# enijkamp/apex_example

Hardware: AMD Instinct MI355X
Metric: images/sec (whole node) ResNet-50 amp O2 (higher is better)
Workload: dtype bf16; 1 GPU; model=resnet50, global_batch=256, per_gpu_batch=256, image_size=224, parallelism=dp1, impl=amd, opt_level=O2, optimizer=FusedSGD(momentum=0.9, wd=5e-5), channels_last=True, fused_bn=True, syncbn=False, force_collectives=False, gemm_1x1=True, hip_graph=False, main_stream_priority=default, deterministic=False

## Files before the change

apex_example_amd/ops/pool.py:

```python
from __future__ import annotations


import torch
import torch.nn as nn
import torch.nn.functional as F

from .. import _native

_FUSE_STEM = True
_FUSE_STEM_BWD = True
_GAP_KERNEL = True


class MaxPool2dNHWCFunction(torch.autograd.Function):
    @staticmethod
    def forward(ctx, x, k, s, p):
        y, idx = _native.require().pool.max_fwd(x, k, s, p)
        ctx.save_for_backward(idx)
        ctx.geom = (x.size(2), x.size(3), k, s, p)
        return y

    @staticmethod
    def backward(ctx, dy):
        (idx,) = ctx.saved_tensors
        H, W, k, s, p = ctx.geom
        return _native.require().pool.max_bwd(dy, idx, H, W, k, s, p), None, None, None


class BNReLUMaxPoolFunction(torch.autograd.Function):

    @staticmethod
    def forward(ctx, x, weight, bias, running_mean, running_var, nbt, eps, momentum, k, s, p,
                pg=None, slab=None, shift=None):
        C = _native.require()
        inv_total = None
        count = x.numel() // x.size(1)
        if pg is None and slab is not None:
            mean, invstd = C.bn.slab_train_stats(slab, count, shift, running_mean, running_var,
                                                 nbt, float(eps), float(momentum))
        elif pg is None:
            mean, invstd = C.bn.train_stats(x, running_mean, running_var, nbt, float(eps),
                                            float(momentum))
        else:
            import torch.distributed as dist
            world = dist.get_world_size(pg)
            packed = (C.bn.slab_packed_stats(slab, count, shift) if slab is not None
                      else C.bn.local_stats_packed(x))
            gathered = torch.empty(world * packed.numel(), dtype=packed.dtype, device=x.device)
            if dist.get_backend(pg) == "nccl":
                dist.all_gather_into_tensor(gathered, packed, group=pg)
            else:
                dist.all_gather(list(gathered.chunk(world)), packed, group=pg)
            mean, invstd, inv_total = C.bn.combine_stats_sync(
                gathered.view(world, -1), float(eps), float(momentum), running_mean,
                running_var, nbt)
        y, idx = C.pool.max_fwd_bn(x, mean, invstd, weight, bias, k, s, p)
        ctx.save_for_backward(x, weight, bias, mean, invstd, idx)
        ctx.geom = (x.size(2), x.size(3), k, s, p)
        ctx.pg, ctx.inv_total = pg, inv_total
        return y

    @staticmethod
    def backward(ctx, dy):
        x, weight, bias, mean, invstd, idx = ctx.saved_tensors
        H, W, k, s, p = ctx.geom
        C = _native.require()
        need_w = weight is not None and (ctx.needs_input_grad[1] or ctx.needs_input_grad[2])
        if (ctx.pg is None and _FUSE_STEM_BWD and (k, s, p) == (3, 2, 1) and x.size(1) == 64
                and x.element_size() == 2 and dy.dtype == x.dtype):
            dbn, slab = C.pool.max_bwd_bn(dy, idx, H, W, x, mean, invstd, weight, bias)
            sum_dy, sum_dy_xmu, gw, gb = C.bn.slab_reduce_grad(slab, invstd, weight, need_w)
            count = float(x.numel() // x.size(1))
        elif ctx.pg is None:
            dbn = C.pool.max_bwd(dy, idx, H, W, k, s, p)
            sum_dy, sum_dy_xmu, gw, gb = C.bn.reduce_grad(dbn, x, mean, invstd, weight, bias,
                                                          None, True, need_w)
            count = float(x.numel() // x.size(1))
        else:
            import torch.distributed as dist
            dbn = C.pool.max_bwd(dy, idx, H, W, k, s, p)
            sum_dy, sum_dy_xmu, gw, gb = C.bn.reduce_grad(dbn, x, mean, invstd, weight, bias,
                                                          None, True, need_w,
                                                          sum_scale=ctx.inv_total)
            n = sum_dy.numel()
            dist.all_reduce(sum_dy.as_strided((2 * n,), (1,)), group=ctx.pg)
            count = 1.0
        dx, _ = C.bn.backward_elemt(dbn, x, mean, invstd, weight, bias, sum_dy, sum_dy_xmu,
                                    count, None, True, False)
        return (dx, gw if need_w else None, gb if need_w else None,
                None, None, None, None, None, None, None, None, None, None, None)


def _stem_pg(bn):
    from .batch_norm import BatchNorm2dReLU

    if type(bn) is BatchNorm2dReLU:
        return None
    from ..parallel.sync_batchnorm import SyncBatchNorm, syncbn_comm_group
    import torch.distributed as dist

    if type(bn) is not SyncBatchNorm or bn.channel_last:
        return False
# ... 71 lines not shown
```

csrc/hip/pool.hip:

```cpp
#include <cstdlib>

#include "amd_dev.h"
#include "amd_kernels.h"
#include "bn_common.h"

namespace amd {

namespace {

constexpr int kPoolThreads = 256;
constexpr int kPoolBNMaxC = 512;

struct PoolBN {
  const float *mean, *invstd, *w, *b;
};

template <typename T, bool VEC, bool BN>
__global__ void __launch_bounds__(kPoolThreads)
    maxpool_fwd_k(const T* __restrict__ x, T* __restrict__ y, uint8_t* __restrict__ idx,
                  int N, int H, int W, int C, int OH, int OW, int k, int s, int p, PoolBN bn) {
  constexpr int V = VEC ? 8 : 1;
  const int CV = C / V;
  const int64_t total = (int64_t)N * OH * OW * CV;
  for (int64_t t = (int64_t)blockIdx.x * blockDim.x + threadIdx.x; t < total;
// ... 182 lines not shown
    for (int i = 0; i < 8; ++i) {
      best[i] = -INFINITY;
      arg[i] = first;
    }
#pragma unroll
    for (int tap = 0; tap < 9; ++tap) {
      if (!((okm >> tap) & 1u)) continue;
      float v[8];
      unpack8_any<T>(raw[tap], v);
      if constexpr (BN) {
#pragma unroll
        for (int i = 0; i < 8; ++i) v[i] = to_f32(from_f32<T>(fmaxf(fmaf(v[i], sc[i], sh[i]), 0.f)));
      }
#pragma unroll
      for (int i = 0; i < 8; ++i) {
        if (v[i] > best[i] || (v[i] != v[i] && best[i] == best[i])) {
          best[i] = v[i];
          arg[i] = tap;
        }
      }
    }
    const int64_t o = (((int64_t)n * OH + oh) * OW + ow) * C + cv * 8;
    store8(y + o, best);
    uint32_t lo = 0, hi = 0;
#pragma unroll
    for (int i = 0; i < 4; ++i) {
      lo |= (uint32_t)(arg[i] & 0xff) << (8 * i);
      hi |= (uint32_t)(arg[i + 4] & 0xff) << (8 * i);
    }
    *reinterpret_cast<uint2*>(idx + o) = make_uint2(lo, hi);
  }
}

template <typename T, bool BNR = false>
__global__ void __launch_bounds__(kPoolThreads)
    maxpool3s2_bwd2_k(const T* __restrict__ dy, const uint8_t* __restrict__ idx,
                      T* __restrict__ dx, int N, int H, int W, int C, int OH, int OW,
                      const T* __restrict__ xin = nullptr, const float* __restrict__ mean = nullptr,
                      const float* __restrict__ invstd = nullptr,
                      const float* __restrict__ bw = nullptr, const float* __restrict__ bb = nullptr,
                      float* __restrict__ slab = nullptr) {
  static_assert(sizeof(T) == 2, "16-bit activations");
  const int CV = C / 8, BH = (H + 1) / 2, BW = (W + 1) / 2;
  const int64_t total = (int64_t)N * BH * BW * CV;
  float mu[8], sc[8], sh[8], s1[8], s2[8];
  if constexpr (BNR) {
    const int cg = (int)(((int64_t)blockIdx.x * blockDim.x + threadIdx.x) % CV);
#pragma unroll
    for (int c = 0; c < 8; ++c) {
      const int ch = cg * 8 + c;
      mu[c] = mean[ch];
      chan_affine(mean, invstd, bw ? bw[ch] : 1.f, bb ? bb[ch] : 0.f, ch, sc[c], sh[c]);
      s1[c] = s2[c] = 0.f;
    }
  }
  for (int64_t t = (int64_t)blockIdx.x * blockDim.x + threadIdx.x; t < total;
       t += (int64_t)gridDim.x * blockDim.x) {
    const int cv = (int)(t % CV);
    int64_t pix = t / CV;
    const int j = (int)(pix % BW);
    pix /= BW;
    const int i = (int)(pix % BH);
    const int n = (int)(pix / BH);
    float g[4][8];
    uint32_t wd[4][2];
    bool ok[4];
#pragma unroll
    for (int a = 0; a < 2; ++a)
#pragma unroll
      for (int b = 0; b < 2; ++b) {
        const int q = a * 2 + b;
        ok[q] = i + a < OH && j + b < OW;
        const int64_t o = (((int64_t)n * OH + (ok[q] ? i + a : i)) * OW + (ok[q] ? j + b : j)) * C +
                          cv * 8;
        unpack8_any<T>(*reinterpret_cast<const p_u32x4*>(dy + o), g[q]);
        const uint2 w2 = *reinterpret_cast<const uint2*>(idx + o);
        wd[q][0] = w2.x;
        wd[q][1] = w2.y;
      }
    auto tap_of = [&](int q, int c) { return (int)((wd[q][c >> 2] >> (8 * (c & 3))) & 0xff); };
#pragma unroll
    for (int dh = 0; dh < 2; ++dh) {
      const int h = 2 * i + dh;
      if (h >= H) continue;
#pragma unroll
      for (int dw = 0; dw < 2; ++dw) {
        const int w = 2 * j + dw;
        if (w >= W) continue;
        float acc[8];
#pragma unroll
        for (int c = 0; c < 8; ++c) acc[c] = 0.f;
#pragma unroll
        for (int a = 0; a < 2; ++a) {
          if (a == 1 && dh == 0) continue;
          const int kh = dh == 0 ? 1 : (a == 0 ? 2 : 0);
#pragma unroll
          for (int b = 0; b < 2; ++b) {
            if (b == 1 && dw == 0) continue;
            const int kw = dw == 0 ? 1 : (b == 0 ? 2 : 0);
            const int q = a * 2 + b;
            if (!ok[q]) continue;
#pragma unroll
            for (int c = 0; c < 8; ++c)
              if (tap_of(q, c) == kh * 3 + kw) acc[c] += g[q][c];
          }
        }
        const int64_t o = (((int64_t)n * H + h) * W + w) * C + cv * 8;
        store8(dx + o, acc);
        if constexpr (BNR) {
          float xv[8];
          unpack8_any<T>(*reinterpret_cast<const p_u32x4*>(xin + o), xv);
#pragma unroll
          for (int c = 0; c < 8; ++c) {
            const float g = to_f32(from_f32<T>(acc[c]));
            const float d = fmaf(xv[c], sc[c], sh[c]) > 0.f ? g : 0.f;
            s1[c] += d;
            s2[c] = fmaf(d, xv[c] - mu[c], s2[c]);
          }
        }
      }
    }
  }
  if constexpr (BNR) {
    __shared__ float red[2][kPoolThreads / 64][64];
    const int lane = threadIdx.x & 63, wv = threadIdx.x >> 6;
#pragma unroll
    for (int c = 0; c < 8; ++c) {
#pragma unroll
      for (int m = 8; m < 64; m <<= 1) {
        s1[c] += __shfl_xor(s1[c], m);
        s2[c] += __shfl_xor(s2[c], m);
      }
    }
    if (lane < 8) {
      const int cg = (int)(((int64_t)blockIdx.x * blockDim.x + threadIdx.x) % CV);
#pragma unroll
      for (int c = 0; c < 8; ++c) {
        red[0][wv][cg * 8 + c] = s1[c];
        red[1][wv][cg * 8 + c] = s2[c];
      }
    }
    __syncthreads();
    if (threadIdx.x < 128) {
      const int q = threadIdx.x >> 6, ch = threadIdx.x & 63;
      float a = 0.f;
#pragma unroll
      for (int w2 = 0; w2 < kPoolThreads / 64; ++w2) a += red[q][w2][ch];
      slab[((int64_t)q * 64 + ch) * gridDim.x + blockIdx.x] = a;
    }
  }
}

template <typename T, bool VEC>
__global__ void __launch_bounds__(kPoolThreads)
    gap_bwd_k(const T* __restrict__ dy, T* __restrict__ dx, int64_t N, int64_t HW, int C,
              float inv_hw) {
// ... 64 lines not shown
    if (vec && with_bn)
      hipLaunchKernelGGL((maxpool_fwd_k<T, true, true>), g, b, 0, st, xp, yp, idx, N, H, W, C,
                         OH, OW, k, s, p, bn);
    else if (vec)
      hipLaunchKernelGGL((maxpool_fwd_k<T, true, false>), g, b, 0, st, xp, yp, idx, N, H, W, C,
                         OH, OW, k, s, p, bn);
    else if (with_bn)
      hipLaunchKernelGGL((maxpool_fwd_k<T, false, true>), g, b, 0, st, xp, yp, idx, N, H, W, C,
                         OH, OW, k, s, p, bn);
    else
      hipLaunchKernelGGL((maxpool_fwd_k<T, false, false>), g, b, 0, st, xp, yp, idx, N, H, W, C,
                         OH, OW, k, s, p, bn);
  });
}

int maxpool_bwd_bn_grid(int N, int H, int W) {
  const int64_t blk = (int64_t)N * ((H + 1) / 2) * ((W + 1) / 2) * 8;
  const int g = pool_grid(blk);
  return g > 2048 ? 2048 : g;
}

bool maxpool2d_nhwc_bwd_bn_ok(int H, int W, int C, int OH, int OW, int k, int s, int p) {
  return C == 64 && stem_ok(k, s, p, H, W, OH, OW);
}

void maxpool2d_nhwc_bwd_bn(const void* dy, const uint8_t* idx, DType t, void* dx, int N, int H,
                           int W, int C, int OH, int OW, const void* x, const float* mean,
                           const float* invstd, const float* bw, const float* bb, float* slab,
                           hipStream_t st) {
  const int grid = maxpool_bwd_bn_grid(N, H, W);
  pool_dispatch(t, [&](auto t0) {
    using T = decltype(t0);
    if constexpr (sizeof(T) == 2) {
      hipLaunchKernelGGL((maxpool3s2_bwd2_k<T, true>), dim3(grid), dim3(kPoolThreads), 0, st,
                         static_cast<const T*>(dy), idx, static_cast<T*>(dx), N, H, W, C, OH, OW,
                         static_cast<const T*>(x), mean, invstd, bw, bb, slab);
    }
  });
}

void maxpool2d_nhwc_bwd(const void* dy, const uint8_t* idx, DType t, void* dx, int N, int H,
                        int W, int C, int OH, int OW, int k, int s, int p, hipStream_t st) {
  const bool vec = C % 8 == 0 && ((uintptr_t)dy % 16) == 0 && ((uintptr_t)dx % 16) == 0 &&
                   ((uintptr_t)idx % 8) == 0;
  const int64_t items = (int64_t)N * H * W * (vec ? C / 8 : C);
  if (items == 0) return;
  pool_dispatch(t, [&](auto t0) {
    using T = decltype(t0);
    if constexpr (sizeof(T) == 2) {
      if (vec && stem_ok(k, s, p, H, W, OH, OW)) {
        const int64_t blk = (int64_t)N * ((H + 1) / 2) * ((W + 1) / 2) * (C / 8);
        hipLaunchKernelGGL((maxpool3s2_bwd2_k<T, false>), dim3(pool_grid(blk)), dim3(kPoolThreads), 0,
                           st, static_cast<const T*>(dy), idx, static_cast<T*>(dx), N, H, W, C,
                           OH, OW);
        return;
      }
    }
    if (vec)
      hipLaunchKernelGGL((maxpool_bwd_k<T, true>), dim3(pool_grid(items)), dim3(kPoolThreads), 0,
                         st, static_cast<const T*>(dy), idx, static_cast<T*>(dx), N, H, W, C, OH,
                         OW, k, s, p);
    else
      hipLaunchKernelGGL((maxpool_bwd_k<T, false>), dim3(pool_grid(items)), dim3(kPoolThreads), 0,
                         st, static_cast<const T*>(dy), idx, static_cast<T*>(dx), N, H, W, C, OH,
                         OW, k, s, p);
  });
}

void gap_nhwc_bwd(const void* dy, DType t, void* dx, int64_t N, int64_t HW, int C,
                  hipStream_t st) {
  const bool vec = C % 8 == 0 && ((uintptr_t)dy % 16) == 0 && ((uintptr_t)dx % 16) == 0;
  const int64_t items = N * HW * (vec ? C / 8 : C);
  if (items == 0) return;
  const float inv_hw = 1.f / (float)HW;
  pool_dispatch(t, [&](auto t0) {
    using T = decltype(t0);
    if (vec)
      hipLaunchKernelGGL((gap_bwd_k<T, true>), dim3(pool_grid(items)), dim3(kPoolThreads), 0, st,
                         static_cast<const T*>(dy), static_cast<T*>(dx), N, HW, C, inv_hw);
    else
      hipLaunchKernelGGL((gap_bwd_k<T, false>), dim3(pool_grid(items)), dim3(kPoolThreads), 0,
                         st, static_cast<const T*>(dy), static_cast<T*>(dx), N, HW, C, inv_hw);
  });
}

// ... 2 lines not shown
```

csrc/include/amd_kernels.h:

```cpp
#pragma once
#include <hip/hip_runtime.h>
#include <stdint.h>
#include "mt_table.h"

namespace amd {

enum class DType : int;

struct ScaleArg {
  const float* ptr;
  float val;
  int invert;
};

void mt_scale(const MTLaunch& L, DType in, DType out, ScaleArg s, int* noop, hipStream_t st);
void mt_check_finite(const MTLaunch& L, DType in, int* noop, hipStream_t st);
void mt_axpby(const MTLaunch& L, DType x, DType y, DType out, ScaleArg a, ScaleArg b,
              int arg_to_check, int* noop, hipStream_t st);
void mt_fill_zero(const MTLaunch& L, DType t, hipStream_t st);
void mt_copy_if(const MTLaunch& L, DType t, const int* flag, hipStream_t st);

void mt_norm_partials(const MTLaunch& L, DType in, int max_norm, float* partials, int* noop,
                      hipStream_t st);
void mt_norm_finalize(const MTLaunch& L, const float* partials, int npart_sets, int max_norm,
// ... 144 lines not shown
                      int64_t C, float eps, float momentum, float* mean_out, float* invstd_out,
                      float* running_mean, DType trm, void* running_var_any, float* var_out,
                      hipStream_t st, long long* nbt = nullptr, float* inv_total = nullptr);
void bn_apply(const void* x, DType tx, const float* mean, const float* invstd,
              const void* weight, const void* bias, DType tw, const void* z, uint8_t* relu_mask,
              void* y, int64_t outer, int64_t C, int64_t inner, int channel_last, int relu,
              hipStream_t st);
void bn_reduce_grad(const void* dy, const void* x, DType tx, const float* mean,
                    const float* invstd, const void* weight, const void* bias, DType tw,
                    int relu, const void* z, const uint8_t* relu_mask, int64_t outer, int64_t C,
                    int64_t inner,
                    int channel_last, float* sum_dy, float* sum_dy_xmu, void* grad_weight,
                    void* grad_bias, float* ws, hipStream_t st,
                    const float* sum_scale = nullptr);
void bn_backward_elemt(const void* dy, const void* x, DType tx, const float* mean,
                       const float* invstd, const void* weight, const void* bias, DType tw,
                       const float* sum_dy, const float* sum_dy_xmu, float inv_count,
                       int relu, const void* z, const uint8_t* relu_mask, void* dx, void* dz,
                       int64_t outer, int64_t C, int64_t inner, int channel_last, hipStream_t st);


void maxpool2d_nhwc_fwd(const void* x, DType t, void* y, uint8_t* idx, int N, int H, int W, int C,
                        int OH, int OW, int k, int s, int p, hipStream_t st,
                        const float* mean = nullptr, const float* invstd = nullptr,
                        const float* bw = nullptr, const float* bb = nullptr);
void maxpool2d_nhwc_bwd(const void* dy, const uint8_t* idx, DType t, void* dx, int N, int H,
                        int W, int C, int OH, int OW, int k, int s, int p, hipStream_t st);
bool maxpool2d_nhwc_bwd_bn_ok(int H, int W, int C, int OH, int OW, int k, int s, int p);
int maxpool_bwd_bn_grid(int N, int H, int W);
void maxpool2d_nhwc_bwd_bn(const void* dy, const uint8_t* idx, DType t, void* dx, int N, int H,
                           int W, int C, int OH, int OW, const void* x, const float* mean,
                           const float* invstd, const float* bw, const float* bb, float* slab,
                           hipStream_t st);
void gap_nhwc_bwd(const void* dy, DType t, void* dx, int64_t N, int64_t HW, int C,
                  hipStream_t st);

struct GemmArgs {
  const void* A;
  const void* B;
  void* C;
  int M, N, K, lda, ldb, ldc;
  const void* bias;
  int bias_f32;
  void* aux;
  float* colsum;
  int tanh;
  int fp16;
  int group_m;
  float* slab;
  const float* shift;
};
bool gemm4w_supported(int M, int N, int K);
void gemm4w(const GemmArgs& a, int epi, hipStream_t st);
struct WgradArgs {
  const void* A;
  const void* B;
  float* P;
  int M, N, lda, ldb;
  int rows;
  int S;
  int fp16;
  int group_m;
  float* colsum = nullptr;
};
bool wgrad4w_supported(int64_t T, int M, int N, int S);
void wgrad4w(const WgradArgs& a, hipStream_t st);
// ... 146 lines not shown
```

csrc/torch/module.cpp:

```cpp
#include <torch/extension.h>

#include "amd_kernels.h"
#include "amp_ops.h"
#include "attn_ops.h"
#include "norm_ops.h"
#include "pool_ops.h"
#include "dense_ops.h"
#include "lt_ops.h"
#include "xent_ops.h"
#include "emb_ops.h"
#include "reducer.h"

#include <hip/hip_runtime_api.h>

#include <cstdint>
#include <vector>

namespace py = pybind11;
using namespace amd;

static at::Tensor flatten_dense(const std::vector<at::Tensor>& ts) {
  std::vector<at::Tensor> flat;
  flat.reserve(ts.size());
  for (auto& t : ts) flat.push_back(t.contiguous().view({-1}));
// ... 83 lines not shown
  dn.def("bias_grad", &bias_grad_op);
  dn.def("gelu_bwd_bias_grad", &gelu_bwd_bias_grad_op);
  dn.def("act_bwd_bias_grad", &act_bwd_bias_grad_op);
  dn.def("gelu", &gelu_fwd_op);
  dn.def("gelu_fwd_lt", &dense_gelu_fwd_op);
  dn.def("dgelu_bgrad_lt", &dense_dgelu_bgrad_op);
  dn.def("lt_cache_clear", &lt_algo_cache_clear);
  dn.def("lt_probe", &lt_probe_op);
  dn.def("wgrad_bgrad_lt", &dense_wgrad_bgrad_op);
  dn.def("gemm4w", &gemm4w_op, py::arg("a"), py::arg("b"), py::arg("epi") = 0,
         py::arg("bias") = py::none(), py::arg("aux") = py::none(), py::arg("want_pre") = false,
         py::arg("tanh") = false, py::arg("bias_grad_dtype") = py::none());
  dn.def("gemm4w_ok", &gemm4w_ok);
  dn.def("wgrad4w", &wgrad4w_op, py::arg("dy"), py::arg("x"), py::arg("splits"),
         py::arg("out_dtype"), py::arg("out") = py::none(), py::arg("accumulate") = true);
  dn.def("wgrad4w_ok", &wgrad4w_ok);
  dn.def("wgrad4w_bias", &wgrad4w_bias_op, py::arg("dy"), py::arg("x"), py::arg("splits"),
         py::arg("out_dtype"), py::arg("out") = py::none(), py::arg("accumulate") = true,
         py::arg("bias_dtype") = at::kFloat);
  auto xe = m.def_submodule("xentropy", "fused softmax cross entropy + label smoothing");
  xe.def("forward", &xentropy_fwd_op);
  xe.def("backward", &xentropy_bwd_op);

  auto emb = m.def_submodule("emb", "deterministic embedding weight gradient (no host sync)");
  emb.def("wgrad", &embedding_wgrad_op, py::arg("idx"), py::arg("dy"), py::arg("V"),
          py::arg("padding_idx"), py::arg("out_dtype"));

  auto pool = m.def_submodule("pool", "NHWC max pooling (gather backward, no atomics)");
  pool.def("max_fwd", &maxpool2d_nhwc_fwd_op);
  pool.def("max_bwd", &maxpool2d_nhwc_bwd_op);
  pool.def("max_bwd_bn", &maxpool2d_nhwc_bwd_bn_op, py::arg("dy"), py::arg("idx"), py::arg("H"),
           py::arg("W"), py::arg("x"), py::arg("mean"), py::arg("invstd"),
           py::arg("weight") = py::none(), py::arg("bias") = py::none());
  pool.def("gap_bwd", &gap_nhwc_bwd_op, py::arg("dy"), py::arg("H"), py::arg("W"));
  pool.def("max_fwd_bn", &maxpool2d_nhwc_bn_fwd_op);
  auto conv = m.def_submodule("conv", "MFMA implicit-GEMM convolutions (NHWC bf16)");
  conv.def("conv_fwd", &conv_nhwc_fwd_op, py::arg("x"), py::arg("w"), py::arg("stride") = 1);
  conv.def("conv_fwd_bnbwd", &conv_nhwc_fwd_bnbwd_op, py::arg("dy"), py::arg("w"),
           py::arg("add"), py::arg("x"), py::arg("rmask"), py::arg("mean"), py::arg("invstd"),
           py::arg("bn_weight"), py::arg("bn_bias"), py::arg("relu_mode"),
           py::arg("add_stride2") = false);
  conv.def("conv_fwd_stats", &conv_nhwc_fwd_stats_op, py::arg("x"), py::arg("w"),
           py::arg("stride") = 1, py::arg("shift") = py::none());
  conv.def("recompute_1x1_ok", &conv1x1_recompute_ok_op, py::arg("M"), py::arg("Cin"),
           py::arg("Cout"));
  conv.def("conv1x1_stats_only", &conv1x1_stats_only_op, py::arg("x"), py::arg("w"),
           py::arg("shift") = py::none());
  conv.def("conv1x1_bn_apply", &conv1x1_bn_apply_op, py::arg("x"), py::arg("w"), py::arg("x3"),
           py::arg("mean"), py::arg("invstd"), py::arg("bn_weight"), py::arg("bn_bias"),
           py::arg("z"));
  conv.def("conv1x1_bn_bwd", &conv1x1_bn_bwd_op, py::arg("x"), py::arg("w"), py::arg("g"),
           py::arg("mean"), py::arg("invstd"), py::arg("bn_weight"), py::arg("sum_dy"),
           py::arg("sum_dy_xmu"), py::arg("count"));
  conv.def("conv_dgrad_s2", &conv_nhwc_dgrad_s2_op);
  conv.def("conv_dgrad_s2_bnbwd", &conv_nhwc_dgrad_s2_bnbwd_op, py::arg("dy"), py::arg("wt"),
           py::arg("H"), py::arg("W"), py::arg("x"), py::arg("rmask"), py::arg("mean"),
           py::arg("invstd"), py::arg("bn_weight"), py::arg("bn_bias"), py::arg("relu_mode"));
  conv.def("conv_wgrad", &conv_nhwc_wgrad_op, py::arg("dy"), py::arg("x"), py::arg("out_dtype"),
           py::arg("algo") = 0, py::arg("stride") = 1, py::arg("ksize") = 3,
           py::arg("out") = py::none(), py::arg("accumulate") = true);
  conv.def("splitk_reduce", &splitk_reduce_op, py::arg("part"), py::arg("out_dtype"),
           py::arg("out") = py::none(), py::arg("accumulate") = true);
  conv.def("stem_pad", &stem_pad_op);
  conv.def("stem_fwd", &stem_fwd_op);
  conv.def("stem_fwd_stats", &stem_fwd_stats_op, py::arg("xp"), py::arg("wk"),
           py::arg("shift") = py::none());
// ... 102 lines not shown
```

csrc/torch/pool_ops.cpp:

```cpp
#include <cstdlib>
#include "pool_ops.h"

#include "common.h"

namespace amd {

namespace {
int64_t out_size(int64_t in, int64_t k, int64_t s, int64_t p) { return (in + 2 * p - k) / s + 1; }
}

std::tuple<at::Tensor, at::Tensor> maxpool2d_nhwc_fwd_op(at::Tensor x, int64_t k, int64_t s,
                                                         int64_t p) {
  return maxpool2d_nhwc_bn_fwd_op(x, c10::nullopt, c10::nullopt, c10::nullopt, c10::nullopt, k, s,
                                  p);
}

std::tuple<at::Tensor, at::Tensor> maxpool2d_nhwc_bn_fwd_op(
    at::Tensor x, c10::optional<at::Tensor> mean, c10::optional<at::Tensor> invstd,
    c10::optional<at::Tensor> w, c10::optional<at::Tensor> b, int64_t k, int64_t s, int64_t p) {
  c10::NoGradGuard no_grad_;
  auto f32 = [&](const c10::optional<at::Tensor>& t) -> const float* {
    if (!t.has_value() || !t->defined()) return nullptr;
    TORCH_CHECK(t->scalar_type() == at::kFloat && t->is_contiguous() && t->is_cuda() &&
                    t->numel() == x.size(1),
// ... 2 lines not shown
  };
  const float* mp = f32(mean);
  const float* ip = f32(invstd);
  TORCH_CHECK((mp == nullptr) == (ip == nullptr), "maxpool BN: mean and invstd go together");
  TORCH_CHECK(x.is_cuda() && x.dim() == 4, "maxpool2d_nhwc: 4-D GPU tensor expected");
  TORCH_CHECK(k >= 1 && k <= 15 && s >= 1 && p >= 0 && p <= k / 2, "unsupported pool geometry");
  x = x.contiguous(at::MemoryFormat::ChannelsLast);
  const int64_t N = x.size(0), C = x.size(1), H = x.size(2), W = x.size(3);
  const int64_t OH = out_size(H, k, s, p), OW = out_size(W, k, s, p);
  TORCH_CHECK(OH > 0 && OW > 0, "pool output is empty");
  auto opt = x.options().memory_format(at::MemoryFormat::ChannelsLast);
  at::Tensor y = at::empty({N, C, OH, OW}, opt);
  at::Tensor idx = at::empty({N, C, OH, OW}, opt.dtype(at::kByte));
  maxpool2d_nhwc_fwd(x.data_ptr(), dtype_of(x), y.data_ptr(), idx.data_ptr<uint8_t>(), (int)N,
                     (int)H, (int)W, (int)C, (int)OH, (int)OW, (int)k, (int)s, (int)p,
                     cur_stream(), mp, ip, f32(w), f32(b));
  return {y, idx};
}

at::Tensor maxpool2d_nhwc_bwd_op(at::Tensor dy, at::Tensor idx, int64_t H, int64_t W, int64_t k,
                                 int64_t s, int64_t p) {
  c10::NoGradGuard no_grad_;
  dy = dy.contiguous(at::MemoryFormat::ChannelsLast);
  idx = idx.contiguous(at::MemoryFormat::ChannelsLast);
  const int64_t N = dy.size(0), C = dy.size(1), OH = dy.size(2), OW = dy.size(3);
  TORCH_CHECK(idx.sizes() == dy.sizes() && idx.scalar_type() == at::kByte, "bad pool index");
  at::Tensor dx = at::empty({N, C, H, W}, dy.options().memory_format(at::MemoryFormat::ChannelsLast));
  maxpool2d_nhwc_bwd(dy.data_ptr(), idx.data_ptr<uint8_t>(), dtype_of(dy), dx.data_ptr(), (int)N,
                     (int)H, (int)W, (int)C, (int)OH, (int)OW, (int)k, (int)s, (int)p,
                     cur_stream());
  return dx;
}

std::tuple<at::Tensor, at::Tensor> maxpool2d_nhwc_bwd_bn_op(at::Tensor dy, at::Tensor idx,
                                                            int64_t H, int64_t W, at::Tensor x,
                                                            at::Tensor mean, at::Tensor invstd,
                                                            c10::optional<at::Tensor> weight,
                                                            c10::optional<at::Tensor> bias) {
  c10::NoGradGuard no_grad_;
  dy = dy.contiguous(at::MemoryFormat::ChannelsLast);
  idx = idx.contiguous(at::MemoryFormat::ChannelsLast);
  const int64_t N = dy.size(0), C = dy.size(1), OH = dy.size(2), OW = dy.size(3);
  TORCH_CHECK(idx.sizes() == dy.sizes() && idx.scalar_type() == at::kByte, "bad pool index");
  TORCH_CHECK(x.is_cuda() && x.dim() == 4 && x.size(0) == N && x.size(1) == C && x.size(2) == H &&
                  x.size(3) == W && x.scalar_type() == dy.scalar_type() &&
                  x.is_contiguous(at::MemoryFormat::ChannelsLast),
              "max_bwd_bn: x must be the pooled BN input [N, C, H, W], channels-last, dy's dtype");
  TORCH_CHECK(dy.element_size() == 2 &&
                  maxpool2d_nhwc_bwd_bn_ok((int)H, (int)W, (int)C, (int)OH, (int)OW, 3, 2, 1),
              "max_bwd_bn: 3x3 / stride-2 / pad-1 pooling of 64 16-bit channels only");
  auto f32c = [&](const at::Tensor& t, const char* what) {
    TORCH_CHECK(t.is_cuda() && t.scalar_type() == at::kFloat && t.numel() == C && t.is_contiguous(),
                "max_bwd_bn: ", what, " must be fp32 [C]");
    return t.data_ptr<float>();
  };
  const float* mp = f32c(mean, "mean");
  const float* ip = f32c(invstd, "invstd");
  const float* wp = weight.has_value() && weight->defined() ? f32c(*weight, "weight") : nullptr;
  const float* bp = bias.has_value() && bias->defined() ? f32c(*bias, "bias") : nullptr;
  at::Tensor dx = at::empty({N, C, H, W}, dy.options().memory_format(at::MemoryFormat::ChannelsLast));
  at::Tensor slab = at::empty({2, C, (int64_t)maxpool_bwd_bn_grid((int)N, (int)H, (int)W)},
                              dy.options().dtype(at::kFloat));
  TORCH_CHECK((uintptr_t)dy.data_ptr() % 16 == 0 && (uintptr_t)dx.data_ptr() % 16 == 0 &&
                  (uintptr_t)x.data_ptr() % 16 == 0 && (uintptr_t)idx.data_ptr() % 8 == 0,
              "max_bwd_bn: 16-byte aligned tensors expected");
  maxpool2d_nhwc_bwd_bn(dy.data_ptr(), idx.data_ptr<uint8_t>(), dtype_of(dy), dx.data_ptr(),
                        (int)N, (int)H, (int)W, (int)C, (int)OH, (int)OW, x.data_ptr(), mp, ip,
                        wp, bp, slab.data_ptr<float>(), cur_stream());
  return {dx, slab};
}

at::Tensor gap_nhwc_bwd_op(at::Tensor dy, int64_t H, int64_t W) {
  c10::NoGradGuard no_grad_;
  TORCH_CHECK(dy.is_cuda() && (dy.dim() == 2 || dy.dim() == 4), "gap_bwd: dy [N, C(, 1, 1)]");
  const int64_t N = dy.size(0), C = dy.size(1);
  TORCH_CHECK(dy.numel() == N * C, "gap_bwd: dy must hold one value per (n, c)");
  dy = dy.reshape({N, C}).contiguous();
  at::Tensor dx =
      at::empty({N, C, H, W}, dy.options().memory_format(at::MemoryFormat::ChannelsLast));
  gap_nhwc_bwd(dy.data_ptr(), dtype_of(dy), dx.data_ptr(), N, H * W, (int)C, cur_stream());
  return dx;
}

}

namespace amd {

at::Tensor conv_nhwc_fwd_op(at::Tensor x, at::Tensor w, int64_t stride) {
  c10::NoGradGuard no_grad_;
  TORCH_CHECK(x.is_cuda() && x.dim() == 4 && w.dim() == 4, "conv: 4-D GPU tensors expected");
  TORCH_CHECK(x.scalar_type() == at::kBFloat16 && w.scalar_type() == at::kBFloat16,
              "conv: bf16 only");
  TORCH_CHECK(stride == 1 || stride == 2, "conv: stride 1 or 2");
  const int64_t N = x.size(0), Cin = x.size(1), H = x.size(2), W = x.size(3);
  const int64_t Cout = w.size(0), k = w.size(2);
  TORCH_CHECK((k == 3 || k == 1) && w.size(3) == k && w.size(1) == Cin, "conv: weight shape");
  const int64_t Ho = (H - 1) / stride + 1, Wo = (W - 1) / stride + 1;
  TORCH_CHECK(conv3x3_nhwc_supported((int)Cin, (int)Cout), "conv: channels must be x64");
  TORCH_CHECK(N * H * W < (int64_t)1 << 31, "conv: too many pixels");
  x = x.contiguous(at::MemoryFormat::ChannelsLast);
  w = w.contiguous(at::MemoryFormat::ChannelsLast);
  at::Tensor y = at::empty({N, Cout, Ho, Wo},
// ... 467 lines not shown
```

csrc/torch/pool_ops.h:

```cpp
#pragma once
#include <ATen/ATen.h>
#include <c10/util/Optional.h>

#include <tuple>

namespace amd {

std::tuple<at::Tensor, at::Tensor> maxpool2d_nhwc_fwd_op(at::Tensor x, int64_t k, int64_t s,
                                                         int64_t p);
std::tuple<at::Tensor, at::Tensor> maxpool2d_nhwc_bn_fwd_op(
    at::Tensor x, c10::optional<at::Tensor> mean, c10::optional<at::Tensor> invstd,
    c10::optional<at::Tensor> w, c10::optional<at::Tensor> b, int64_t k, int64_t s, int64_t p);
at::Tensor maxpool2d_nhwc_bwd_op(at::Tensor dy, at::Tensor idx, int64_t H, int64_t W, int64_t k,
                                 int64_t s, int64_t p);
at::Tensor gap_nhwc_bwd_op(at::Tensor dy, int64_t H, int64_t W);

at::Tensor conv_nhwc_fwd_op(at::Tensor x, at::Tensor w, int64_t stride);
std::tuple<at::Tensor, at::Tensor> conv_nhwc_fwd_stats_op(at::Tensor x, at::Tensor w,
                                                          int64_t stride,
                                                          c10::optional<at::Tensor> shift);
std::tuple<at::Tensor, at::Tensor> conv_nhwc_fwd_bnbwd_op(
    at::Tensor dy, at::Tensor w, c10::optional<at::Tensor> add, at::Tensor xbn,
    c10::optional<at::Tensor> rmask, at::Tensor mean, at::Tensor invstd,
    c10::optional<at::Tensor> bn_w, c10::optional<at::Tensor> bn_b, int64_t relu_mode,
    bool add_stride2 = false);
bool conv1x1_recompute_ok_op(int64_t M, int64_t Cin, int64_t Cout);
std::tuple<at::Tensor, at::Tensor> conv1x1_stats_only_op(at::Tensor x, at::Tensor w,
                                                         c10::optional<at::Tensor> shift);
std::tuple<at::Tensor, at::Tensor> conv1x1_bn_apply_op(at::Tensor x, at::Tensor w, at::Tensor x3,
                                                       at::Tensor mean, at::Tensor invstd,
                                                       at::Tensor bn_w, at::Tensor bn_b,
                                                       at::Tensor z);
at::Tensor conv1x1_bn_bwd_op(at::Tensor x, at::Tensor w, at::Tensor g, at::Tensor mean,
                             at::Tensor invstd, at::Tensor bn_w, at::Tensor sum_dy,
                             at::Tensor sum_dy_xmu, double count);
at::Tensor conv_nhwc_dgrad_s2_op(at::Tensor dy, at::Tensor wt, int64_t H, int64_t W);
at::Tensor conv_nhwc_wgrad_op(at::Tensor dy, at::Tensor x, at::ScalarType out_dtype, int64_t algo,
                              int64_t stride, int64_t ksize, c10::optional<at::Tensor> out, bool accumulate = true);
at::Tensor splitk_reduce_op(at::Tensor part, at::ScalarType out_dtype,
                            c10::optional<at::Tensor> out_acc, bool accumulate = true);
at::Tensor stem_pad_op(at::Tensor x);
at::Tensor stem_fwd_op(at::Tensor xp, at::Tensor wk);
std::tuple<at::Tensor, at::Tensor> conv_nhwc_dgrad_s2_bnbwd_op(
    at::Tensor dy, at::Tensor wt, int64_t H, int64_t W, at::Tensor xbn,
    c10::optional<at::Tensor> rmask, at::Tensor mean, at::Tensor invstd,
    c10::optional<at::Tensor> bn_w, c10::optional<at::Tensor> bn_b, int64_t relu_mode);
std::tuple<at::Tensor, at::Tensor> maxpool2d_nhwc_bwd_bn_op(at::Tensor dy, at::Tensor idx,
                                                            int64_t H, int64_t W, at::Tensor x,
                                                            at::Tensor mean, at::Tensor invstd,
                                                            c10::optional<at::Tensor> weight,
                                                            c10::optional<at::Tensor> bias);
std::tuple<at::Tensor, at::Tensor> stem_fwd_stats_op(at::Tensor xp, at::Tensor wk,
                                                     c10::optional<at::Tensor> shift);
at::Tensor stem_wgrad_op(at::Tensor xp, at::Tensor dy);
at::Tensor conv3x3_rot_weight_op(at::Tensor w);
at::Tensor conv1x1_transpose_weight_op(at::Tensor w);
std::vector<at::Tensor> conv_prep_weights_op(std::vector<at::Tensor> ws);

}
```

Baseline: 12830 images/s.

## Recompute stem maxpool backward inside BN dx kernel instead of materializing dbn

Splits the stem maxpool+BN-ReLU backward into a sums-only pass (no dbn write) and a second pass that recomputes the pooled gradient and applies the BN backward elementwise directly to produce dx. This removes the write and re-read of the full-resolution dbn tensor and the separate backward_elemt kernel. In exchange, dy, idx and x are read twice and the scatter logic runs twice.

```diff
diff --git a/apex_example_amd/ops/pool.py b/apex_example_amd/ops/pool.py
--- a/apex_example_amd/ops/pool.py
+++ b/apex_example_amd/ops/pool.py
@@ -9,6 +9,7 @@
 
 _FUSE_STEM = True
 _FUSE_STEM_BWD = True
+_FUSE_STEM_DX = True
 _GAP_KERNEL = True
 
 
@@ -66,8 +67,16 @@
         H, W, k, s, p = ctx.geom
         C = _native.require()
         need_w = weight is not None and (ctx.needs_input_grad[1] or ctx.needs_input_grad[2])
-        if (ctx.pg is None and _FUSE_STEM_BWD and (k, s, p) == (3, 2, 1) and x.size(1) == 64
-                and x.element_size() == 2 and dy.dtype == x.dtype):
+        stem = (ctx.pg is None and _FUSE_STEM_BWD and (k, s, p) == (3, 2, 1) and x.size(1) == 64
+                and x.element_size() == 2 and dy.dtype == x.dtype)
+        if stem and _FUSE_STEM_DX:
+            slab = C.pool.max_bwd_bn_sums(dy, idx, H, W, x, mean, invstd, weight, bias)
+            sum_dy, sum_dy_xmu, gw, gb = C.bn.slab_reduce_grad(slab, invstd, weight, need_w)
+            dx = C.pool.max_bwd_bn_dx(dy, idx, H, W, x, mean, invstd, weight, bias, sum_dy,
+                                      sum_dy_xmu, float(x.numel() // x.size(1)))
+            return (dx, gw if need_w else None, gb if need_w else None,
+                    None, None, None, None, None, None, None, None, None, None, None)
+        if stem:
             dbn, slab = C.pool.max_bwd_bn(dy, idx, H, W, x, mean, invstd, weight, bias)
             sum_dy, sum_dy_xmu, gw, gb = C.bn.slab_reduce_grad(slab, invstd, weight, need_w)
             count = float(x.numel() // x.size(1))
diff --git a/csrc/hip/pool.hip b/csrc/hip/pool.hip
--- a/csrc/hip/pool.hip
+++ b/csrc/hip/pool.hip
@@ -238,19 +238,26 @@
   }
 }
 
-template <typename T, bool BNR = false>
+enum PoolBwd : int { kBwdPlain = 0, kBwdBNR = 1, kBwdBNSums = 2, kBwdBNDX = 3 };
+
+template <typename T, int MODE = kBwdPlain>
 __global__ void __launch_bounds__(kPoolThreads)
     maxpool3s2_bwd2_k(const T* __restrict__ dy, const uint8_t* __restrict__ idx,
                       T* __restrict__ dx, int N, int H, int W, int C, int OH, int OW,
                       const T* __restrict__ xin = nullptr, const float* __restrict__ mean = nullptr,
                       const float* __restrict__ invstd = nullptr,
                       const float* __restrict__ bw = nullptr, const float* __restrict__ bb = nullptr,
-                      float* __restrict__ slab = nullptr) {
+                      float* __restrict__ slab = nullptr,
+                      const float* __restrict__ sum_dy = nullptr,
+                      const float* __restrict__ sum_dy_xmu = nullptr, float inv_n = 0.f) {
+  constexpr bool SUMS = MODE == kBwdBNR || MODE == kBwdBNSums;
+  constexpr bool BNDX = MODE == kBwdBNDX;
+  constexpr bool XUP = MODE == kBwdBNSums || BNDX;
   static_assert(sizeof(T) == 2, "16-bit activations");
   const int CV = C / 8, BH = (H + 1) / 2, BW = (W + 1) / 2;
   const int64_t total = (int64_t)N * BH * BW * CV;
-  float mu[8], sc[8], sh[8], s1[8], s2[8];
-  if constexpr (BNR) {
+  float mu[8], sc[8], sh[8], s1[8], s2[8], k1[8], k2[8], k3[8];
+  if constexpr (SUMS) {
     const int cg = (int)(((int64_t)blockIdx.x * blockDim.x + threadIdx.x) % CV);
 #pragma unroll
     for (int c = 0; c < 8; ++c) {
@@ -258,6 +265,17 @@
       mu[c] = mean[ch];
       chan_affine(mean, invstd, bw ? bw[ch] : 1.f, bb ? bb[ch] : 0.f, ch, sc[c], sh[c]);
       s1[c] = s2[c] = 0.f;
+    }
+  }
+  if constexpr (BNDX) {
+    const int cg = (int)(((int64_t)blockIdx.x * blockDim.x + threadIdx.x) % CV);
+#pragma unroll
+    for (int c = 0; c < 8; ++c) {
+      const int ch = cg * 8 + c;
+      const float wc = bw ? bw[ch] : 1.f;
+      chan_affine(mean, invstd, wc, bb ? bb[ch] : 0.f, ch, sc[c], sh[c]);
+      bn_bwd_consts(invstd[ch], wc, mean[ch], sum_dy[ch], sum_dy_xmu[ch], inv_n, k1[c], k2[c],
+                    k3[c]);
     }
   }
   for (int64_t t = (int64_t)blockIdx.x * blockDim.x + threadIdx.x; t < total;
@@ -284,6 +302,16 @@
         wd[q][0] = w2.x;
         wd[q][1] = w2.y;
       }
+    p_u32x4 xr[XUP ? 4 : 1];
+    if constexpr (XUP) {
+#pragma unroll
+      for (int q = 0; q < 4; ++q) {
+        const int h = 2 * i + (q >> 1), w = 2 * j + (q & 1);
+        const bool in = h < H && w < W;
+        xr[q] = *reinterpret_cast<const p_u32x4*>(
+            xin + (((int64_t)n * H + (in ? h : 2 * i)) * W + (in ? w : 2 * j)) * C + cv * 8);
+      }
+    }
     auto tap_of = [&](int q, int c) { return (int)((wd[q][c >> 2] >> (8 * (c & 3))) & 0xff); };
 #pragma unroll
     for (int dh = 0; dh < 2; ++dh) {
@@ -312,10 +340,11 @@
           }
         }
         const int64_t o = (((int64_t)n * H + h) * W + w) * C + cv * 8;
-        store8(dx + o, acc);
-        if constexpr (BNR) {
+        if constexpr (MODE == kBwdPlain || MODE == kBwdBNR) store8(dx + o, acc);
+        if constexpr (SUMS) {
           float xv[8];
-          unpack8_any<T>(*reinterpret_cast<const p_u32x4*>(xin + o), xv);
+          if constexpr (XUP) unpack8_any<T>(xr[dh * 2 + dw], xv);
+          else unpack8_any<T>(*reinterpret_cast<const p_u32x4*>(xin + o), xv);
 #pragma unroll
           for (int c = 0; c < 8; ++c) {
             const float g = to_f32(from_f32<T>(acc[c]));
@@ -324,10 +353,22 @@
             s2[c] = fmaf(d, xv[c] - mu[c], s2[c]);
           }
         }
-      }
-    }
-  }
-  if constexpr (BNR) {
+        if constexpr (BNDX) {
+          float xv[8], r[8];
+          if constexpr (XUP) unpack8_any<T>(xr[dh * 2 + dw], xv);
+          else unpack8_any<T>(*reinterpret_cast<const p_u32x4*>(xin + o), xv);
+#pragma unroll
+          for (int c = 0; c < 8; ++c) {
+            const float g = to_f32(from_f32<T>(acc[c]));
+            const float d = fmaf(xv[c], sc[c], sh[c]) > 0.f ? g : 0.f;
+            r[c] = bn_bwd_elem(d, xv[c], k1[c], k2[c], k3[c]);
+          }
+          store8(dx + o, r);
+        }
+      }
+    }
+  }
+  if constexpr (SUMS) {
     __shared__ float red[2][kPoolThreads / 64][64];
     const int lane = threadIdx.x & 63, wv = threadIdx.x >> 6;
 #pragma unroll
@@ -458,9 +499,31 @@
   pool_dispatch(t, [&](auto t0) {
     using T = decltype(t0);
     if constexpr (sizeof(T) == 2) {
-      hipLaunchKernelGGL((maxpool3s2_bwd2_k<T, true>), dim3(grid), dim3(kPoolThreads), 0, st,
+      if (dx)
+        hipLaunchKernelGGL((maxpool3s2_bwd2_k<T, kBwdBNR>), dim3(grid), dim3(kPoolThreads), 0, st,
+                           static_cast<const T*>(dy), idx, static_cast<T*>(dx), N, H, W, C, OH,
+                           OW, static_cast<const T*>(x), mean, invstd, bw, bb, slab);
+      else
+        hipLaunchKernelGGL((maxpool3s2_bwd2_k<T, kBwdBNSums>), dim3(grid), dim3(kPoolThreads), 0,
+                           st, static_cast<const T*>(dy), idx, static_cast<T*>(nullptr), N, H, W,
+                           C, OH, OW, static_cast<const T*>(x), mean, invstd, bw, bb, slab);
+    }
+  });
+}
+
+void maxpool2d_nhwc_bwd_bn_dx(const void* dy, const uint8_t* idx, DType t, void* dx, int N, int H,
+                              int W, int C, int OH, int OW, const void* x, const float* mean,
+                              const float* invstd, const float* bw, const float* bb,
+                              const float* sum_dy, const float* sum_dy_xmu, float inv_n,
+                              hipStream_t st) {
+  const int grid = maxpool_bwd_bn_grid(N, H, W);
+  pool_dispatch(t, [&](auto t0) {
+    using T = decltype(t0);
+    if constexpr (sizeof(T) == 2) {
+      hipLaunchKernelGGL((maxpool3s2_bwd2_k<T, kBwdBNDX>), dim3(grid), dim3(kPoolThreads), 0, st,
                          static_cast<const T*>(dy), idx, static_cast<T*>(dx), N, H, W, C, OH, OW,
-                         static_cast<const T*>(x), mean, invstd, bw, bb, slab);
+                         static_cast<const T*>(x), mean, invstd, bw, bb,
+                         static_cast<float*>(nullptr), sum_dy, sum_dy_xmu, inv_n);
     }
   });
 }
@@ -476,7 +539,7 @@
     if constexpr (sizeof(T) == 2) {
       if (vec && stem_ok(k, s, p, H, W, OH, OW)) {
         const int64_t blk = (int64_t)N * ((H + 1) / 2) * ((W + 1) / 2) * (C / 8);
-        hipLaunchKernelGGL((maxpool3s2_bwd2_k<T, false>), dim3(pool_grid(blk)), dim3(kPoolThreads), 0,
+        hipLaunchKernelGGL((maxpool3s2_bwd2_k<T, kBwdPlain>), dim3(pool_grid(blk)), dim3(kPoolThreads), 0,
                            st, static_cast<const T*>(dy), idx, static_cast<T*>(dx), N, H, W, C,
                            OH, OW);
         return;
diff --git a/csrc/include/amd_kernels.h b/csrc/include/amd_kernels.h
--- a/csrc/include/amd_kernels.h
+++ b/csrc/include/amd_kernels.h
@@ -200,6 +200,11 @@
                            int W, int C, int OH, int OW, const void* x, const float* mean,
                            const float* invstd, const float* bw, const float* bb, float* slab,
                            hipStream_t st);
+void maxpool2d_nhwc_bwd_bn_dx(const void* dy, const uint8_t* idx, DType t, void* dx, int N, int H,
+                              int W, int C, int OH, int OW, const void* x, const float* mean,
+                              const float* invstd, const float* bw, const float* bb,
+                              const float* sum_dy, const float* sum_dy_xmu, float inv_n,
+                              hipStream_t st);
 void gap_nhwc_bwd(const void* dy, DType t, void* dx, int64_t N, int64_t HW, int C,
                   hipStream_t st);
 
diff --git a/csrc/torch/module.cpp b/csrc/torch/module.cpp
--- a/csrc/torch/module.cpp
+++ b/csrc/torch/module.cpp
@@ -139,6 +139,13 @@
   pool.def("max_bwd_bn", &maxpool2d_nhwc_bwd_bn_op, py::arg("dy"), py::arg("idx"), py::arg("H"),
            py::arg("W"), py::arg("x"), py::arg("mean"), py::arg("invstd"),
            py::arg("weight") = py::none(), py::arg("bias") = py::none());
+  pool.def("max_bwd_bn_sums", &maxpool2d_nhwc_bwd_bn_sums_op, py::arg("dy"), py::arg("idx"),
+           py::arg("H"), py::arg("W"), py::arg("x"), py::arg("mean"), py::arg("invstd"),
+           py::arg("weight") = py::none(), py::arg("bias") = py::none());
+  pool.def("max_bwd_bn_dx", &maxpool2d_nhwc_bwd_bn_dx_op, py::arg("dy"), py::arg("idx"),
+           py::arg("H"), py::arg("W"), py::arg("x"), py::arg("mean"), py::arg("invstd"),
+           py::arg("weight"), py::arg("bias"), py::arg("sum_dy"), py::arg("sum_dy_xmu"),
+           py::arg("count"));
   pool.def("gap_bwd", &gap_nhwc_bwd_op, py::arg("dy"), py::arg("H"), py::arg("W"));
   pool.def("max_fwd_bn", &maxpool2d_nhwc_bn_fwd_op);
   auto conv = m.def_submodule("conv", "MFMA implicit-GEMM convolutions (NHWC bf16)");
diff --git a/csrc/torch/pool_ops.cpp b/csrc/torch/pool_ops.cpp
--- a/csrc/torch/pool_ops.cpp
+++ b/csrc/torch/pool_ops.cpp
@@ -58,12 +58,20 @@
   return dx;
 }
 
-std::tuple<at::Tensor, at::Tensor> maxpool2d_nhwc_bwd_bn_op(at::Tensor dy, at::Tensor idx,
-                                                            int64_t H, int64_t W, at::Tensor x,
-                                                            at::Tensor mean, at::Tensor invstd,
-                                                            c10::optional<at::Tensor> weight,
-                                                            c10::optional<at::Tensor> bias) {
-  c10::NoGradGuard no_grad_;
+namespace {
+struct StemBwd {
+  int N, C, H, W, OH, OW;
+  const float *mean, *invstd, *w, *b;
+};
+const float* stem_f32c(const at::Tensor& t, int64_t C, const char* op, const char* what) {
+  TORCH_CHECK(t.is_cuda() && t.scalar_type() == at::kFloat && t.numel() == C && t.is_contiguous(),
+              op, ": ", what, " must be fp32 [C]");
+  return t.data_ptr<float>();
+}
+StemBwd stem_bwd_check(at::Tensor& dy, at::Tensor& idx, int64_t H, int64_t W, const at::Tensor& x,
+                       const at::Tensor& mean, const at::Tensor& invstd,
+                       const c10::optional<at::Tensor>& weight,
+                       const c10::optional<at::Tensor>& bias, const char* op) {
   dy = dy.contiguous(at::MemoryFormat::ChannelsLast);
   idx = idx.contiguous(at::MemoryFormat::ChannelsLast);
   const int64_t N = dy.size(0), C = dy.size(1), OH = dy.size(2), OW = dy.size(3);
@@ -71,29 +79,76 @@
   TORCH_CHECK(x.is_cuda() && x.dim() == 4 && x.size(0) == N && x.size(1) == C && x.size(2) == H &&
                   x.size(3) == W && x.scalar_type() == dy.scalar_type() &&
                   x.is_contiguous(at::MemoryFormat::ChannelsLast),
-              "max_bwd_bn: x must be the pooled BN input [N, C, H, W], channels-last, dy's dtype");
+              op, ": x must be the pooled BN input [N, C, H, W], channels-last, dy's dtype");
   TORCH_CHECK(dy.element_size() == 2 &&
                   maxpool2d_nhwc_bwd_bn_ok((int)H, (int)W, (int)C, (int)OH, (int)OW, 3, 2, 1),
-              "max_bwd_bn: 3x3 / stride-2 / pad-1 pooling of 64 16-bit channels only");
-  auto f32c = [&](const at::Tensor& t, const char* what) {
-    TORCH_CHECK(t.is_cuda() && t.scalar_type() == at::kFloat && t.numel() == C && t.is_contiguous(),
-                "max_bwd_bn: ", what, " must be fp32 [C]");
-    return t.data_ptr<float>();
-  };
-  const float* mp = f32c(mean, "mean");
-  const float* ip = f32c(invstd, "invstd");
-  const float* wp = weight.has_value() && weight->defined() ? f32c(*weight, "weight") : nullptr;
-  const float* bp = bias.has_value() && bias->defined() ? f32c(*bias, "bias") : nullptr;
-  at::Tensor dx = at::empty({N, C, H, W}, dy.options().memory_format(at::MemoryFormat::ChannelsLast));
-  at::Tensor slab = at::empty({2, C, (int64_t)maxpool_bwd_bn_grid((int)N, (int)H, (int)W)},
-                              dy.options().dtype(at::kFloat));
-  TORCH_CHECK((uintptr_t)dy.data_ptr() % 16 == 0 && (uintptr_t)dx.data_ptr() % 16 == 0 &&
-                  (uintptr_t)x.data_ptr() % 16 == 0 && (uintptr_t)idx.data_ptr() % 8 == 0,
-              "max_bwd_bn: 16-byte aligned tensors expected");
-  maxpool2d_nhwc_bwd_bn(dy.data_ptr(), idx.data_ptr<uint8_t>(), dtype_of(dy), dx.data_ptr(),
-                        (int)N, (int)H, (int)W, (int)C, (int)OH, (int)OW, x.data_ptr(), mp, ip,
-                        wp, bp, slab.data_ptr<float>(), cur_stream());
+              op, ": 3x3 / stride-2 / pad-1 pooling of 64 16-bit channels only");
+  StemBwd r{(int)N, (int)C, (int)H, (int)W, (int)OH, (int)OW};
+  r.mean = stem_f32c(mean, C, op, "mean");
+  r.invstd = stem_f32c(invstd, C, op, "invstd");
+  r.w = weight.has_value() && weight->defined() ? stem_f32c(*weight, C, op, "weight") : nullptr;
+  r.b = bias.has_value() && bias->defined() ? stem_f32c(*bias, C, op, "bias") : nullptr;
+  TORCH_CHECK((uintptr_t)dy.data_ptr() % 16 == 0 && (uintptr_t)x.data_ptr() % 16 == 0 &&
+                  (uintptr_t)idx.data_ptr() % 8 == 0,
+              op, ": 16-byte aligned tensors expected");
+  return r;
+}
+at::Tensor stem_bwd_out(const at::Tensor& dy, const StemBwd& r, const char* op) {
+  at::Tensor dx = at::empty({r.N, r.C, r.H, r.W},
+                            dy.options().memory_format(at::MemoryFormat::ChannelsLast));
+  TORCH_CHECK((uintptr_t)dx.data_ptr() % 16 == 0, op, ": 16-byte aligned tensors expected");
+  return dx;
+}
+at::Tensor stem_bwd_slab(const at::Tensor& dy, const StemBwd& r) {
+  return at::empty({2, r.C, (int64_t)maxpool_bwd_bn_grid(r.N, r.H, r.W)},
+                   dy.options().dtype(at::kFloat));
+}
+}
+
+std::tuple<at::Tensor, at::Tensor> maxpool2d_nhwc_bwd_bn_op(at::Tensor dy, at::Tensor idx,
+                                                            int64_t H, int64_t W, at::Tensor x,
+                                                            at::Tensor mean, at::Tensor invstd,
+                                                            c10::optional<at::Tensor> weight,
+                                                            c10::optional<at::Tensor> bias) {
+  c10::NoGradGuard no_grad_;
+  const StemBwd r = stem_bwd_check(dy, idx, H, W, x, mean, invstd, weight, bias, "max_bwd_bn");
+  at::Tensor dx = stem_bwd_out(dy, r, "max_bwd_bn");
+  at::Tensor slab = stem_bwd_slab(dy, r);
+  maxpool2d_nhwc_bwd_bn(dy.data_ptr(), idx.data_ptr<uint8_t>(), dtype_of(dy), dx.data_ptr(), r.N,
+                        r.H, r.W, r.C, r.OH, r.OW, x.data_ptr(), r.mean, r.invstd, r.w, r.b,
+                        slab.data_ptr<float>(), cur_stream());
   return {dx, slab};
+}
+
+at::Tensor maxpool2d_nhwc_bwd_bn_sums_op(at::Tensor dy, at::Tensor idx, int64_t H, int64_t W,
+                                         at::Tensor x, at::Tensor mean, at::Tensor invstd,
+                                         c10::optional<at::Tensor> weight,
+                                         c10::optional<at::Tensor> bias) {
+  c10::NoGradGuard no_grad_;
+  const StemBwd r =
+      stem_bwd_check(dy, idx, H, W, x, mean, invstd, weight, bias, "max_bwd_bn_sums");
+  at::Tensor slab = stem_bwd_slab(dy, r);
+  maxpool2d_nhwc_bwd_bn(dy.data_ptr(), idx.data_ptr<uint8_t>(), dtype_of(dy), nullptr, r.N, r.H,
+                        r.W, r.C, r.OH, r.OW, x.data_ptr(), r.mean, r.invstd, r.w, r.b,
+                        slab.data_ptr<float>(), cur_stream());
+  return slab;
+}
+
+at::Tensor maxpool2d_nhwc_bwd_bn_dx_op(at::Tensor dy, at::Tensor idx, int64_t H, int64_t W,
+                                       at::Tensor x, at::Tensor mean, at::Tensor invstd,
+                                       c10::optional<at::Tensor> weight,
+                                       c10::optional<at::Tensor> bias, at::Tensor sum_dy,
+                                       at::Tensor sum_dy_xmu, double count) {
+  c10::NoGradGuard no_grad_;
+  const StemBwd r = stem_bwd_check(dy, idx, H, W, x, mean, invstd, weight, bias, "max_bwd_bn_dx");
+  const float* sd = stem_f32c(sum_dy, r.C, "max_bwd_bn_dx", "sum_dy");
+  const float* sx = stem_f32c(sum_dy_xmu, r.C, "max_bwd_bn_dx", "sum_dy_xmu");
+  TORCH_CHECK(count > 0, "max_bwd_bn_dx: count must be positive");
+  at::Tensor dx = stem_bwd_out(dy, r, "max_bwd_bn_dx");
+  maxpool2d_nhwc_bwd_bn_dx(dy.data_ptr(), idx.data_ptr<uint8_t>(), dtype_of(dy), dx.data_ptr(),
+                           r.N, r.H, r.W, r.C, r.OH, r.OW, x.data_ptr(), r.mean, r.invstd, r.w,
+                           r.b, sd, sx, (float)(1.0 / count), cur_stream());
+  return dx;
 }
 
 at::Tensor gap_nhwc_bwd_op(at::Tensor dy, int64_t H, int64_t W) {
diff --git a/csrc/torch/pool_ops.h b/csrc/torch/pool_ops.h
--- a/csrc/torch/pool_ops.h
+++ b/csrc/torch/pool_ops.h
@@ -50,6 +50,15 @@
                                                             at::Tensor mean, at::Tensor invstd,
                                                             c10::optional<at::Tensor> weight,
                                                             c10::optional<at::Tensor> bias);
+at::Tensor maxpool2d_nhwc_bwd_bn_sums_op(at::Tensor dy, at::Tensor idx, int64_t H, int64_t W,
+                                         at::Tensor x, at::Tensor mean, at::Tensor invstd,
+                                         c10::optional<at::Tensor> weight,
+                                         c10::optional<at::Tensor> bias);
+at::Tensor maxpool2d_nhwc_bwd_bn_dx_op(at::Tensor dy, at::Tensor idx, int64_t H, int64_t W,
+                                       at::Tensor x, at::Tensor mean, at::Tensor invstd,
+                                       c10::optional<at::Tensor> weight,
+                                       c10::optional<at::Tensor> bias, at::Tensor sum_dy,
+                                       at::Tensor sum_dy_xmu, double count);
 std::tuple<at::Tensor, at::Tensor> stem_fwd_stats_op(at::Tensor xp, at::Tensor wk,
                                                      c10::optional<at::Tensor> shift);
 at::Tensor stem_wgrad_op(at::Tensor xp, at::Tensor dy);
```

Measured after the change: 12910 images/s (median of 6 runs). About the same (+0.6%).
